# VinAIResearch/DiMSUM

Measured on AMD Instinct MI355X. Metric: denoiser-fwd latents/sec, higher is better.
Workload: dtype f32; 1 GPU; DiM-L/2 denoiser forward, 256px (4x32x32 latents, 256 tokens), 256 latents per GPU, random-init weights (reference init, zero tensors re-drawn N(0, 0.02^2)); global_batch=256, parallelism=dp1 (replicas, independent latents), launch=eager, matmul_policy=f16s (see notes.matmul_policy)

## Files before the change

### dimsum_amd/csrc/xattn_common.hpp

```cpp
#pragma once
#include "common.hpp"

namespace dimsum {

typedef float f4 __attribute__((ext_vector_type(4)));
typedef __bf16 bf16x8 __attribute__((ext_vector_type(8)));
struct alignas(16) u4v { unsigned w[4]; };

__device__ __forceinline__ bf16x8 as_bf16x8(const u4v &v) { return __builtin_bit_cast(bf16x8, v); }

__device__ __forceinline__ float quad_max(float x) {
    auto r = __builtin_amdgcn_permlane16_swap(__float_as_uint(x), __float_as_uint(x), false, false);
    x = fmaxf(__uint_as_float(r[0]), __uint_as_float(r[1]));
    r = __builtin_amdgcn_permlane32_swap(__float_as_uint(x), __float_as_uint(x), false, false);
    return fmaxf(__uint_as_float(r[0]), __uint_as_float(r[1]));
}
__device__ __forceinline__ float quad_sum(float x) {
    auto r = __builtin_amdgcn_permlane16_swap(__float_as_uint(x), __float_as_uint(x), false, false);
    x = __uint_as_float(r[0]) + __uint_as_float(r[1]);
    r = __builtin_amdgcn_permlane32_swap(__float_as_uint(x), __float_as_uint(x), false, false);
    return __uint_as_float(r[0]) + __uint_as_float(r[1]);
}

__device__ __forceinline__ f4 mfma_split(const u4v &ah, const u4v &al, const u4v &bh, const u4v &bl, f4 acc) {
    acc = __builtin_amdgcn_mfma_f32_16x16x32_bf16(as_bf16x8(al), as_bf16x8(bh), acc, 0, 0, 0);
    acc = __builtin_amdgcn_mfma_f32_16x16x32_bf16(as_bf16x8(ah), as_bf16x8(bl), acc, 0, 0, 0);
    acc = __builtin_amdgcn_mfma_f32_16x16x32_bf16(as_bf16x8(ah), as_bf16x8(bh), acc, 0, 0, 0);
    return acc;
}

__device__ __forceinline__ int cslot(int kappa) { return 8 * ((kappa & 15) >> 2) + (kappa & 3) + 4 * (kappa >> 4); }

__device__ __forceinline__ void split_c2(const f4 &t0, const f4 &t1, u4v &hi, u4v &lo) {
    split2(t0[0], t0[1], hi.w[0], lo.w[0]);
    split2(t0[2], t0[3], hi.w[1], lo.w[1]);
    split2(t1[0], t1[1], hi.w[2], lo.w[2]);
    split2(t1[2], t1[3], hi.w[3], lo.w[3]);
}

typedef _Float16 f16x8 __attribute__((ext_vector_type(8)));
__device__ __forceinline__ f16x8 as_f16x8(const u4v &v) { return __builtin_bit_cast(f16x8, v); }
__device__ __forceinline__ unsigned pack_h2(float a, float b) {
    const __half2 h = __floats2half2_rn(a, b);
    return __builtin_bit_cast(unsigned, h);
}
template <bool F16> struct Frag { u4v h, l; };
template <> struct Frag<true> { u4v h; };
template <bool F16> __device__ __forceinline__ void frag_put2(Frag<F16> &f, int i, float x0, float x1) {
    if constexpr (F16) f.h.w[i] = pack_h2(x0, x1);
    else split2(x0, x1, f.h.w[i], f.l.w[i]);
}
template <bool F16> __device__ __forceinline__ Frag<F16> frag_ld(const unsigned short *hi, const unsigned short *lo, int idx) {
    Frag<F16> f;
    f.h = *reinterpret_cast<const u4v *>(&hi[idx]);
    if constexpr (!F16) f.l = *reinterpret_cast<const u4v *>(&lo[idx]);
    return f;
}
template <bool F16> __device__ __forceinline__ f4 frag_mfma(const Frag<F16> &a, const Frag<F16> &b, f4 acc) {
    if constexpr (F16) return __builtin_amdgcn_mfma_f32_16x16x32_f16(as_f16x8(a.h), as_f16x8(b.h), acc, 0, 0, 0);
    else return mfma_split(a.h, a.l, b.h, b.l, acc);
}
template <bool F16> __device__ __forceinline__ Frag<F16> frag_c2(const f4 &t0, const f4 &t1) {
    Frag<F16> f;
    frag_put2<F16>(f, 0, t0[0], t0[1]); frag_put2<F16>(f, 1, t0[2], t0[3]);
    frag_put2<F16>(f, 2, t1[0], t1[1]); frag_put2<F16>(f, 3, t1[2], t1[3]);
    return f;
}
template <bool F16> __device__ __forceinline__ void img_st4(unsigned short *hi, unsigned short *lo, int idx, const float4 &v) {
    if constexpr (F16) *reinterpret_cast<uint2 *>(&hi[idx]) = make_uint2(pack_h2(v.x, v.y), pack_h2(v.z, v.w));
    else {
        unsigned h0, l0, h1, l1;
        split2(v.x, v.y, h0, l0); split2(v.z, v.w, h1, l1);
        *reinterpret_cast<uint2 *>(&hi[idx]) = make_uint2(h0, h1); *reinterpret_cast<uint2 *>(&lo[idx]) = make_uint2(l0, l1);
    }
}
template <bool F16> __device__ __forceinline__ void img_st2(unsigned short *hi, unsigned short *lo, int idx, float x0, float x1) {
    if constexpr (F16) *reinterpret_cast<unsigned *>(&hi[idx]) = pack_h2(x0, x1);
    else {
        unsigned h0, l0;
        split2(x0, x1, h0, l0);
        *reinterpret_cast<unsigned *>(&hi[idx]) = h0; *reinterpret_cast<unsigned *>(&lo[idx]) = l0;
    }
}
template <bool F16> __device__ __forceinline__ void img_zero(unsigned short *hi, unsigned short *lo, int idx) {
    hi[idx] = 0;
    if constexpr (!F16) lo[idx] = 0;
}
__device__ __forceinline__ float row_pow2_scale(float amax) {
    const unsigned e = min((__float_as_uint(amax) >> 23) & 0xffu, 248u);
    return __uint_as_float((249u - e) << 23);
}
constexpr int kPShift = 8;

__device__ __forceinline__ int xcd_group_blocks(int idx, int nblocks, int per_group) {
    if (((nblocks / per_group) & 7) != 0 || nblocks % per_group != 0) return idx;
    const int x = idx & 7, j = idx >> 3;
    return ((j / per_group) * 8 + x) * per_group + (j % per_group);
}

}
```

### dimsum_amd/csrc/xattn_fusion_f16.hip

```cpp
#include <type_traits>

#include "xattn_common.hpp"

namespace dimsum {

constexpr int kKT16 = 64;
constexpr int kQW16 = 16;

template <int HD, int QT, bool kIn16>
__global__ __launch_bounds__(256, (QT == 2 && HD <= 64) ? 3 : 2) void xattn_fusion_fwd_f16_kernel(const dimsum_xattn_params_t p) {
    constexpr int EP = (HD + 31) / 32 * 32;
    constexpr int EC = EP / 32;
    constexpr int ET = (HD + 15) / 16;
    constexpr int KS = EP + 8;
    constexpr int VS = kKT16 + 8;
    static_assert(HD % 8 == 0 && (KS / 8) % 2 == 1 && (VS / 8) % 2 == 1, "layout");
    auto flip = [](int row) { return (((row & 15) + 4) & 8); };
    __shared__ __attribute__((aligned(16))) unsigned short Kh[kKT16 * KS];
    __shared__ __attribute__((aligned(16))) unsigned short Vh[ET * 16 * VS];
    __shared__ float red[8];

    const int tid = threadIdx.x, lane = tid & 63, wave = tid >> 6;
    const int L = p.seqlen, H = p.heads;
    const int qblocks = (L + 64 * QT - 1) / (64 * QT);
    int idx = xcd_group_blocks(blockIdx.x, (int)gridDim.x, qblocks);
    const int qb = idx % qblocks; idx /= qblocks;
    const int ndir = p.n_dirs == 1 ? 1 : 2;
    const int dir = idx % ndir; idx /= ndir;
    const int h = idx % H;
    const int b = idx / H;
    const int C = H * HD;
    const bool kv_from_1 = dir == 1 || ndir == 1;
    using In = typename std::conditional<kIn16, __half, float>::type;
    const In *qsrc = reinterpret_cast<const In *>(dir == 0 ? p.qkv1_ptr : p.qkv2_ptr) + (int64_t)b * p.qkv_batch_stride + h * HD;
    const In *kvsrc = reinterpret_cast<const In *>(kv_from_1 ? p.qkv1_ptr : p.qkv2_ptr) + (int64_t)b * p.qkv_batch_stride + h * HD;
    const In *ksrc = kvsrc + C, *vsrc = kvsrc + 2 * C;
    const int64_t ts = p.qkv_token_stride;
    const float *qbv = reinterpret_cast<const float *>(dir == 0 ? p.bias1_ptr : p.bias2_ptr);
    const float *kvb = reinterpret_cast<const float *>(kv_from_1 ? p.bias1_ptr : p.bias2_ptr);
    const float *qbias = qbv ? qbv + h * HD : nullptr;
    const float *kbias = kvb ? kvb + C + h * HD : nullptr, *vbias = kvb ? kvb + 2 * C + h * HD : nullptr;

    float kv_scale, kv_inv, o_scale = 1.f, o_inv = 1.f;
    const float *bnd = reinterpret_cast<const float *>(p.kv_bound_ptr);
    const float *i1 = reinterpret_cast<const float *>(p.x1_inv_ptr) + (int64_t)b * L;
    const float *i2 = ndir == 2 ? reinterpret_cast<const float *>(p.x2_inv_ptr) + (int64_t)b * L : i1;
    {
        float m1 = 0.f, m2 = 0.f;
        for (int t = tid; t < L; t += 256) { m1 = fmaxf(m1, i1[t]); m2 = fmaxf(m2, i2[t]); }
        m1 = wave_allmax(m1); m2 = wave_allmax(m2);
        if (lane == 0) { red[wave] = m1; red[4 + wave] = m2; }
        __syncthreads();
        m1 = fmaxf(fmaxf(red[0], red[1]), fmaxf(red[2], red[3]));
        m2 = fmaxf(fmaxf(red[4], red[5]), fmaxf(red[6], red[7]));
        const float b1 = 2.0f * (32768.0f * m1 * bnd[0] + bnd[1]), b2 = ndir == 2 ? 2.0f * (32768.0f * m2 * bnd[2] + bnd[3]) : b1;
        f16s_scales(kv_from_1 ? b1 : b2, kv_scale, kv_inv);
        if (p.out_split3 == 2) f16s_scales(fmaxf(b1, b2), o_scale, o_inv);
    }

    const int qi = lane & 15, kg = lane >> 4;
    int q_tok[QT];
    u4v qh[QT][EC];
    float cq[QT];
#pragma unroll
    for (int t = 0; t < QT; ++t) {
        q_tok[t] = qb * (64 * QT) + (wave * QT + t) * kQW16 + qi;
        const int q_ld = min(q_tok[t], L - 1);
        if constexpr (kIn16) {
            float qs, qinv;
            const float xinv = (dir == 0 ? i1 : i2)[q_ld];
            f16s_scales(2.0f * (32768.0f * xinv * bnd[dir == 0 ? 0 : 2] + bnd[dir == 0 ? 1 : 3]), qs, qinv);
            cq[t] = fmaxf(p.scale * kLog2e * qinv * kv_inv, 1.17549435e-38f);
#pragma unroll
            for (int c = 0; c < EC; ++c) {
                const int e0 = 32 * c + 8 * kg;
                qh[t][c] = u4v{{0u, 0u, 0u, 0u}};
                if (e0 < HD) qh[t][c] = *reinterpret_cast<const u4v *>(qsrc + (int64_t)q_ld * ts + e0);
            }
            continue;
        }
        float v[EC][8], qm = 0.f;
#pragma unroll
        for (int c = 0; c < EC; ++c)
#pragma unroll
            for (int half = 0; half < 2; ++half) {
                const int e0 = 32 * c + 8 * kg + 4 * half;
                float4 tq = make_float4(0.f, 0.f, 0.f, 0.f);
                if (e0 < HD) {
                    tq = *reinterpret_cast<const float4 *>(reinterpret_cast<const float *>(qsrc) + (int64_t)q_ld * ts + e0);
                    if (qbias) { const float4 bq = *reinterpret_cast<const float4 *>(qbias + e0); tq.x += bq.x; tq.y += bq.y; tq.z += bq.z; tq.w += bq.w; }
                }
                v[c][4 * half + 0] = tq.x; v[c][4 * half + 1] = tq.y; v[c][4 * half + 2] = tq.z; v[c][4 * half + 3] = tq.w;
                qm = fmaxf(fmaxf(qm, fmaxf(fabsf(tq.x), fabsf(tq.y))), fmaxf(fabsf(tq.z), fabsf(tq.w)));
            }
        float qs, qinv;
        f16s_scales(quad_max(qm), qs, qinv);
        cq[t] = fmaxf(p.scale * kLog2e * qinv * kv_inv, 1.17549435e-38f);
#pragma unroll
        for (int c = 0; c < EC; ++c)
#pragma unroll
            for (int i = 0; i < 4; ++i) qh[t][c].w[i] = pack_h2(v[c][2 * i] * qs, v[c][2 * i + 1] * qs);
    }
    if constexpr (EP > HD) {
        for (int i = tid; i < kKT16 * (EP - HD); i += 256) { const int key = i / (EP - HD), e = (HD + i % (EP - HD)) ^ flip(key); Kh[key * KS + e] = 0; }
    }
    if constexpr (ET * 16 > HD) {
        for (int i = tid; i < (ET * 16 - HD) * kKT16; i += 256) { const int e = HD + i / kKT16, k = (i % kKT16) ^ flip(e); Vh[e * VS + k] = 0; }
    }

    f4 o[QT][ET];
    float m_run[QT], l_run[QT];
#pragma unroll
    for (int t = 0; t < QT; ++t) {
        m_run[t] = -1e30f; l_run[t] = 0.f;
#pragma unroll
        for (int e = 0; e < ET; ++e) o[t][e] = f4{0.f, 0.f, 0.f, 0.f};
    }

    constexpr int kItems = (kKT16 / 2) * (HD / 4), kIters = (kItems + 255) / 256;
    constexpr int kItems16 = (kKT16 / 2) * (HD / 8), kIters16 = (kItems16 + 255) / 256;
    for (int k0 = 0; k0 < L; k0 += kKT16) {
        __syncthreads();
        if constexpr (kIn16) {
#pragma unroll
            for (int it = 0; it < kIters16; ++it) {
                const int i = tid + it * 256;
                if (kItems16 % 256 != 0 && i >= kItems16) continue;
                const int kp = i / (HD / 8), e8 = i - kp * (HD / 8), key = 2 * kp;
                const int tok0 = min(k0 + key, L - 1), tok1 = min(k0 + key + 1, L - 1);
                const u4v ka = *reinterpret_cast<const u4v *>(ksrc + (int64_t)tok0 * ts + e8 * 8), kb = *reinterpret_cast<const u4v *>(ksrc + (int64_t)tok1 * ts + e8 * 8);
                const u4v va = *reinterpret_cast<const u4v *>(vsrc + (int64_t)tok0 * ts + e8 * 8), vb = *reinterpret_cast<const u4v *>(vsrc + (int64_t)tok1 * ts + e8 * 8);
                const int ke = (e8 * 8) ^ flip(key);
                *reinterpret_cast<u4v *>(&Kh[key * KS + ke]) = ka;
                *reinterpret_cast<u4v *>(&Kh[(key + 1) * KS + ke]) = kb;
                const int kap = key & 31, pos = (key & ~31) + 8 * ((kap & 15) >> 2) + (kap & 3) + 4 * (kap >> 4);
#pragma unroll
                for (int j = 0; j < 4; ++j) {
                    *reinterpret_cast<unsigned *>(&Vh[(e8 * 8 + 2 * j) * VS + (pos ^ flip(e8 * 8 + 2 * j))]) = __builtin_amdgcn_perm(vb.w[j], va.w[j], 0x05040100u);
                    *reinterpret_cast<unsigned *>(&Vh[(e8 * 8 + 2 * j + 1) * VS + (pos ^ flip(e8 * 8 + 2 * j + 1))]) = __builtin_amdgcn_perm(vb.w[j], va.w[j], 0x07060302u);
                }
            }
        } else {
#pragma unroll
        for (int it = 0; it < kIters; ++it) {
            const int i = tid + it * 256;
            if (kItems % 256 != 0 && i >= kItems) continue;
            const int kp = i / (HD / 4), e4 = i - kp * (HD / 4), key = 2 * kp;
            const int tok0 = min(k0 + key, L - 1), tok1 = min(k0 + key + 1, L - 1);
            const float *kf = reinterpret_cast<const float *>(ksrc), *vf = reinterpret_cast<const float *>(vsrc);
            float4 ka = *reinterpret_cast<const float4 *>(kf + (int64_t)tok0 * ts + e4 * 4), kb = *reinterpret_cast<const float4 *>(kf + (int64_t)tok1 * ts + e4 * 4);
            float4 va = *reinterpret_cast<const float4 *>(vf + (int64_t)tok0 * ts + e4 * 4), vb = *reinterpret_cast<const float4 *>(vf + (int64_t)tok1 * ts + e4 * 4);
            if (kbias) {
                const float4 bk = *reinterpret_cast<const float4 *>(kbias + e4 * 4), bv = *reinterpret_cast<const float4 *>(vbias + e4 * 4);
                ka.x += bk.x; ka.y += bk.y; ka.z += bk.z; ka.w += bk.w; kb.x += bk.x; kb.y += bk.y; kb.z += bk.z; kb.w += bk.w;
                va.x += bv.x; va.y += bv.y; va.z += bv.z; va.w += bv.w; vb.x += bv.x; vb.y += bv.y; vb.z += bv.z; vb.w += bv.w;
            }
            const int ke = (e4 * 4) ^ flip(key);
            *reinterpret_cast<uint2 *>(&Kh[key * KS + ke]) = make_uint2(pack_h2(ka.x * kv_scale, ka.y * kv_scale), pack_h2(ka.z * kv_scale, ka.w * kv_scale));
            *reinterpret_cast<uint2 *>(&Kh[(key + 1) * KS + ke]) = make_uint2(pack_h2(kb.x * kv_scale, kb.y * kv_scale), pack_h2(kb.z * kv_scale, kb.w * kv_scale));
            const int kap = key & 31, pos = (key & ~31) + 8 * ((kap & 15) >> 2) + (kap & 3) + 4 * (kap >> 4);
            const float a4[4] = {va.x, va.y, va.z, va.w}, b4[4] = {vb.x, vb.y, vb.z, vb.w};
#pragma unroll
            for (int e = 0; e < 4; ++e)
                *reinterpret_cast<unsigned *>(&Vh[(e4 * 4 + e) * VS + (pos ^ flip(e4 * 4))]) = pack_h2(a4[e] * kv_scale, b4[e] * kv_scale);
        }
        }
        __syncthreads();

        f4 s[QT][4];
#pragma unroll
        for (int kt = 0; kt < 4; ++kt) {
            const int krow = (kt * 16 + qi) * KS + ((8 * kg) ^ flip(qi));
#pragma unroll
            for (int t = 0; t < QT; ++t) s[t][kt] = f4{0.f, 0.f, 0.f, 0.f};
#pragma unroll
            for (int c = 0; c < EC; ++c) {
                const u4v kh = *reinterpret_cast<const u4v *>(&Kh[krow + 32 * c]);
#pragma unroll
                for (int t = 0; t < QT; ++t) s[t][kt] = __builtin_amdgcn_mfma_f32_16x16x32_f16(as_f16x8(kh), as_f16x8(qh[t][c]), s[t][kt], 0, 0, 0);
            }
        }
        u4v ph[QT][2];
#pragma unroll
        for (int t = 0; t < QT; ++t) {
            if (k0 + kKT16 > L) {
#pragma unroll
                for (int kt = 0; kt < 4; ++kt)
#pragma unroll
                    for (int r = 0; r < 4; ++r)
                        if (k0 + kt * 16 + kg * 4 + r >= L) s[t][kt][r] = -INFINITY;
            }
            float mx = -INFINITY;
#pragma unroll
            for (int kt = 0; kt < 4; ++kt)
#pragma unroll
                for (int r = 0; r < 4; ++r) mx = fmaxf(mx, s[t][kt][r]);
            mx = quad_max(mx) * cq[t];
            const float m_new = fmaxf(m_run[t], mx);
            const float alpha = fast_exp2(m_run[t] - m_new);
            float rs = 0.f;
#pragma unroll
            for (int kt = 0; kt < 4; ++kt)
#pragma unroll
                for (int r = 0; r < 4; ++r) { s[t][kt][r] = fast_exp2(fmaf(s[t][kt][r], cq[t], -m_new)); rs += s[t][kt][r]; }
            rs = quad_sum(rs);
            l_run[t] = l_run[t] * alpha + rs;
            m_run[t] = m_new;
#pragma unroll
            for (int e = 0; e < ET; ++e) o[t][e] *= alpha;
#pragma unroll
            for (int c = 0; c < 2; ++c) {
                ph[t][c].w[0] = pack_h2(s[t][2 * c][0], s[t][2 * c][1]);
                ph[t][c].w[1] = pack_h2(s[t][2 * c][2], s[t][2 * c][3]);
                ph[t][c].w[2] = pack_h2(s[t][2 * c + 1][0], s[t][2 * c + 1][1]);
                ph[t][c].w[3] = pack_h2(s[t][2 * c + 1][2], s[t][2 * c + 1][3]);
            }
        }
#pragma unroll
        for (int e = 0; e < ET; ++e) {
            const int vrow = (e * 16 + qi) * VS + ((8 * kg) ^ flip(qi));
#pragma unroll
            for (int c = 0; c < 2; ++c) {
                const u4v vh = *reinterpret_cast<const u4v *>(&Vh[vrow + 32 * c]);
#pragma unroll
                for (int t = 0; t < QT; ++t) o[t][e] = __builtin_amdgcn_mfma_f32_16x16x32_f16(as_f16x8(vh), as_f16x8(ph[t][c]), o[t][e], 0, 0, 0);
            }
        }
    }

#pragma unroll
    for (int t = 0; t < QT; ++t) {
        const bool valid = q_tok[t] < L;
        const float inv = kv_inv / l_run[t];
        const int64_t row_off = (int64_t)b * p.out_batch_stride + (int64_t)min(q_tok[t], L - 1) * p.out_token_stride;
        if (p.out_split3 == 2) {
            __half *img = reinterpret_cast<__half *>(p.out_ptr) + row_off + dir * C + h * HD;
            const float sc = inv * o_scale;
            constexpr int kTr = ET >= 4 ? 4 : 0;
            if constexpr (kTr == 4) {
                float x[4][4];
#pragma unroll
                for (int e = 0; e < 4; ++e)
#pragma unroll
                    for (int r = 0; r < 4; ++r) x[e][r] = o[t][e][r] * sc;
#pragma unroll
                for (int r = 0; r < 4; ++r) {
                    { auto q = __builtin_amdgcn_permlane32_swap(__float_as_uint(x[0][r]), __float_as_uint(x[2][r]), false, false); x[0][r] = __uint_as_float(q[0]); x[2][r] = __uint_as_float(q[1]); }
                    { auto q = __builtin_amdgcn_permlane32_swap(__float_as_uint(x[1][r]), __float_as_uint(x[3][r]), false, false); x[1][r] = __uint_as_float(q[0]); x[3][r] = __uint_as_float(q[1]); }
                    { auto q = __builtin_amdgcn_permlane16_swap(__float_as_uint(x[0][r]), __float_as_uint(x[1][r]), false, false); x[0][r] = __uint_as_float(q[0]); x[1][r] = __uint_as_float(q[1]); }
                    { auto q = __builtin_amdgcn_permlane16_swap(__float_as_uint(x[2][r]), __float_as_uint(x[3][r]), false, false); x[2][r] = __uint_as_float(q[0]); x[3][r] = __uint_as_float(q[1]); }
                }
                if (valid) {
                    __half *d0 = img + 16 * kg;
                    *reinterpret_cast<uint4 *>(d0) = make_uint4(pack_h2(x[0][0], x[0][1]), pack_h2(x[0][2], x[0][3]), pack_h2(x[1][0], x[1][1]), pack_h2(x[1][2], x[1][3]));
                    *reinterpret_cast<uint4 *>(d0 + 8) = make_uint4(pack_h2(x[2][0], x[2][1]), pack_h2(x[2][2], x[2][3]), pack_h2(x[3][0], x[3][1]), pack_h2(x[3][2], x[3][3]));
                }
            }
            if (valid) {
#pragma unroll
                for (int e = kTr; e < ET; ++e) {
                    const int e0 = e * 16 + kg * 4;
                    if (e0 < HD) *reinterpret_cast<uint2 *>(img + e0) = make_uint2(pack_h2(o[t][e][0] * sc, o[t][e][1] * sc), pack_h2(o[t][e][2] * sc, o[t][e][3] * sc));
                }
                if (dir == 0 && h == 0 && kg == 0) reinterpret_cast<float *>(p.out_inv_ptr)[(int64_t)b * L + q_tok[t]] = o_inv;
            }
        } else if (valid) {
            float *dst = reinterpret_cast<float *>(p.out_ptr) + row_off + dir * C + h * HD;
#pragma unroll
            for (int e = 0; e < ET; ++e) {
                const int e0 = e * 16 + kg * 4;
                if (e0 < HD) *reinterpret_cast<float4 *>(dst + e0) = make_float4(o[t][e][0] * inv, o[t][e][1] * inv, o[t][e][2] * inv, o[t][e][3] * inv);
            }
        }
        if (valid && p.lse_ptr && kg == 0)
            reinterpret_cast<float *>(p.lse_ptr)[(((int64_t)b * ndir + dir) * H + h) * L + q_tok[t]] = (m_run[t] + __builtin_amdgcn_logf(l_run[t])) * kLn2;
    }
}

int launch_xattn_f16(const dimsum_xattn_params_t &p, hipStream_t s) {
    const bool self_attn = p.n_dirs == 1;
    const bool two = p.seqlen >= 128;
    const int64_t nblk = (int64_t)p.batch * p.heads * (self_attn ? 1 : 2) * ((p.seqlen + (two ? 127 : 63)) / (two ? 128 : 64));
    if (nblk > 0x7fffffff) return DIMSUM_ERR_SHAPE;
    const dim3 grid((unsigned)nblk), block(256);
#define DIMSUM_XF16(HDV)                                                                                \
    if (p.qkv_f16) {                                                                                    \
        if (two) hipLaunchKernelGGL((xattn_fusion_fwd_f16_kernel<HDV, 2, true>), grid, block, 0, s, p); \
        else hipLaunchKernelGGL((xattn_fusion_fwd_f16_kernel<HDV, 1, true>), grid, block, 0, s, p);     \
    } else if (two) hipLaunchKernelGGL((xattn_fusion_fwd_f16_kernel<HDV, 2, false>), grid, block, 0, s, p); \
    else hipLaunchKernelGGL((xattn_fusion_fwd_f16_kernel<HDV, 1, false>), grid, block, 0, s, p)
    switch (p.head_dim) {
        case 24: DIMSUM_XF16(24); break;
        case 32: DIMSUM_XF16(32); break;
        case 48: DIMSUM_XF16(48); break;
        case 64: DIMSUM_XF16(64); break;
        case 72: DIMSUM_XF16(72); break;
        default: return DIMSUM_ERR_SHAPE;
    }
#undef DIMSUM_XF16
    return launch_status();
}

}
```

Measured before the change: 3590 latents/s.

## Store V row-major in LDS and read with ds_read_tr16 transpose loads

V tiles are now written to shared memory in natural key-major layout with a power-of-two XOR swizzle, replacing the scattered per-element transposed stores. The PV MFMA operand is fetched with the hardware transpose-read instruction ds_read_tr16_b64, two loads per fragment. This cuts the staging cost of V (fewer, wider LDS stores, no perm packing) and also raises occupancy to 3 blocks for the f16-input QT=2 variant. The risk is register pressure from the new occupancy bound and bank conflicts if the swizzle does not match the transposed-read pattern.

```diff
diff --git a/dimsum_amd/csrc/xattn_common.hpp b/dimsum_amd/csrc/xattn_common.hpp
--- a/dimsum_amd/csrc/xattn_common.hpp
+++ b/dimsum_amd/csrc/xattn_common.hpp
@@ -1,5 +1,6 @@
 #pragma once
 #include "common.hpp"
+#include "xattn_layout.hpp"
 
 namespace dimsum {
 
@@ -43,6 +44,11 @@
 __device__ __forceinline__ unsigned pack_h2(float a, float b) {
     const __half2 h = __floats2half2_rn(a, b);
     return __builtin_bit_cast(unsigned, h);
+}
+typedef short s16x4 __attribute__((ext_vector_type(4)));
+__device__ __forceinline__ uint2 lds_read_tr16(const unsigned short *p) {
+    typedef __attribute__((address_space(3))) s16x4 lds_s16x4;
+    return __builtin_bit_cast(uint2, __builtin_amdgcn_ds_read_tr16_b64_v4i16((lds_s16x4 *)p));
 }
 template <bool F16> struct Frag { u4v h, l; };
 template <> struct Frag<true> { u4v h; };
diff --git a/dimsum_amd/csrc/xattn_fusion_f16.hip b/dimsum_amd/csrc/xattn_fusion_f16.hip
--- a/dimsum_amd/csrc/xattn_fusion_f16.hip
+++ b/dimsum_amd/csrc/xattn_fusion_f16.hip
@@ -8,16 +8,15 @@
 constexpr int kQW16 = 16;
 
 template <int HD, int QT, bool kIn16>
-__global__ __launch_bounds__(256, (QT == 2 && HD <= 64) ? 3 : 2) void xattn_fusion_fwd_f16_kernel(const dimsum_xattn_params_t p) {
+__global__ __launch_bounds__(256, (QT == 2 && (HD <= 64 || kIn16)) ? 3 : 2) void xattn_fusion_fwd_f16_kernel(const dimsum_xattn_params_t p) {
     constexpr int EP = (HD + 31) / 32 * 32;
     constexpr int EC = EP / 32;
     constexpr int ET = (HD + 15) / 16;
-    constexpr int KS = EP + 8;
-    constexpr int VS = kKT16 + 8;
-    static_assert(HD % 8 == 0 && (KS / 8) % 2 == 1 && (VS / 8) % 2 == 1, "layout");
-    auto flip = [](int row) { return (((row & 15) + 4) & 8); };
+    constexpr int KS = xattn_k_stride(EP);
+    constexpr int VS = xattn_v_stride(ET);
+    static_assert(HD % 8 == 0 && (KS / 8) % 2 == 1 && xattn_v_layout_ok(ET), "layout");
     __shared__ __attribute__((aligned(16))) unsigned short Kh[kKT16 * KS];
-    __shared__ __attribute__((aligned(16))) unsigned short Vh[ET * 16 * VS];
+    __shared__ __attribute__((aligned(16))) unsigned short Vh[kKT16 * VS];
     __shared__ float red[8];
 
     const int tid = threadIdx.x, lane = tid & 63, wave = tid >> 6;
@@ -102,10 +101,10 @@
             for (int i = 0; i < 4; ++i) qh[t][c].w[i] = pack_h2(v[c][2 * i] * qs, v[c][2 * i + 1] * qs);
     }
     if constexpr (EP > HD) {
-        for (int i = tid; i < kKT16 * (EP - HD); i += 256) { const int key = i / (EP - HD), e = (HD + i % (EP - HD)) ^ flip(key); Kh[key * KS + e] = 0; }
+        for (int i = tid; i < kKT16 * (EP - HD); i += 256) { const int key = i / (EP - HD); Kh[xattn_k_idx(EP, key, HD + i % (EP - HD))] = 0; }
     }
     if constexpr (ET * 16 > HD) {
-        for (int i = tid; i < (ET * 16 - HD) * kKT16; i += 256) { const int e = HD + i / kKT16, k = (i % kKT16) ^ flip(e); Vh[e * VS + k] = 0; }
+        for (int i = tid; i < kKT16 * (ET * 16 - HD); i += 256) { const int key = i / (ET * 16 - HD); Vh[xattn_v_idx(ET, key, HD + i % (ET * 16 - HD))] = 0; }
     }
 
     f4 o[QT][ET];
@@ -126,43 +125,35 @@
             for (int it = 0; it < kIters16; ++it) {
                 const int i = tid + it * 256;
                 if (kItems16 % 256 != 0 && i >= kItems16) continue;
-                const int kp = i / (HD / 8), e8 = i - kp * (HD / 8), key = 2 * kp;
+                const int key = xattn_stage16_key(HD, i, 0), e = xattn_stage16_e(HD, i);
                 const int tok0 = min(k0 + key, L - 1), tok1 = min(k0 + key + 1, L - 1);
-                const u4v ka = *reinterpret_cast<const u4v *>(ksrc + (int64_t)tok0 * ts + e8 * 8), kb = *reinterpret_cast<const u4v *>(ksrc + (int64_t)tok1 * ts + e8 * 8);
-                const u4v va = *reinterpret_cast<const u4v *>(vsrc + (int64_t)tok0 * ts + e8 * 8), vb = *reinterpret_cast<const u4v *>(vsrc + (int64_t)tok1 * ts + e8 * 8);
-                const int ke = (e8 * 8) ^ flip(key);
-                *reinterpret_cast<u4v *>(&Kh[key * KS + ke]) = ka;
-                *reinterpret_cast<u4v *>(&Kh[(key + 1) * KS + ke]) = kb;
-                const int kap = key & 31, pos = (key & ~31) + 8 * ((kap & 15) >> 2) + (kap & 3) + 4 * (kap >> 4);
-#pragma unroll
-                for (int j = 0; j < 4; ++j) {
-                    *reinterpret_cast<unsigned *>(&Vh[(e8 * 8 + 2 * j) * VS + (pos ^ flip(e8 * 8 + 2 * j))]) = __builtin_amdgcn_perm(vb.w[j], va.w[j], 0x05040100u);
-                    *reinterpret_cast<unsigned *>(&Vh[(e8 * 8 + 2 * j + 1) * VS + (pos ^ flip(e8 * 8 + 2 * j + 1))]) = __builtin_amdgcn_perm(vb.w[j], va.w[j], 0x07060302u);
-                }
+                const u4v ka = *reinterpret_cast<const u4v *>(ksrc + (int64_t)tok0 * ts + e), kb = *reinterpret_cast<const u4v *>(ksrc + (int64_t)tok1 * ts + e);
+                const u4v va = *reinterpret_cast<const u4v *>(vsrc + (int64_t)tok0 * ts + e), vb = *reinterpret_cast<const u4v *>(vsrc + (int64_t)tok1 * ts + e);
+                *reinterpret_cast<u4v *>(&Kh[xattn_k_idx(EP, key, e)]) = ka;
+                *reinterpret_cast<u4v *>(&Kh[xattn_k_idx(EP, key + 1, e)]) = kb;
+                *reinterpret_cast<u4v *>(&Vh[xattn_v_idx(ET, key, e)]) = va;
+                *reinterpret_cast<u4v *>(&Vh[xattn_v_idx(ET, key + 1, e)]) = vb;
             }
         } else {
 #pragma unroll
         for (int it = 0; it < kIters; ++it) {
             const int i = tid + it * 256;
             if (kItems % 256 != 0 && i >= kItems) continue;
-            const int kp = i / (HD / 4), e4 = i - kp * (HD / 4), key = 2 * kp;
+            const int key = xattn_stage32_key(HD, i, 0), e = xattn_stage32_e(HD, i);
             const int tok0 = min(k0 + key, L - 1), tok1 = min(k0 + key + 1, L - 1);
             const float *kf = reinterpret_cast<const float *>(ksrc), *vf = reinterpret_cast<const float *>(vsrc);
-            float4 ka = *reinterpret_cast<const float4 *>(kf + (int64_t)tok0 * ts + e4 * 4), kb = *reinterpret_cast<const float4 *>(kf + (int64_t)tok1 * ts + e4 * 4);
-            float4 va = *reinterpret_cast<const float4 *>(vf + (int64_t)tok0 * ts + e4 * 4), vb = *reinterpret_cast<const float4 *>(vf + (int64_t)tok1 * ts + e4 * 4);
+            float4 ka = *reinterpret_cast<const float4 *>(kf + (int64_t)tok0 * ts + e), kb = *reinterpret_cast<const float4 *>(kf + (int64_t)tok1 * ts + e);
+            float4 va = *reinterpret_cast<const float4 *>(vf + (int64_t)tok0 * ts + e), vb = *reinterpret_cast<const float4 *>(vf + (int64_t)tok1 * ts + e);
             if (kbias) {
-                const float4 bk = *reinterpret_cast<const float4 *>(kbias + e4 * 4), bv = *reinterpret_cast<const float4 *>(vbias + e4 * 4);
+                const float4 bk = *reinterpret_cast<const float4 *>(kbias + e), bv = *reinterpret_cast<const float4 *>(vbias + e);
                 ka.x += bk.x; ka.y += bk.y; ka.z += bk.z; ka.w += bk.w; kb.x += bk.x; kb.y += bk.y; kb.z += bk.z; kb.w += bk.w;
                 va.x += bv.x; va.y += bv.y; va.z += bv.z; va.w += bv.w; vb.x += bv.x; vb.y += bv.y; vb.z += bv.z; vb.w += bv.w;
             }
-            const int ke = (e4 * 4) ^ flip(key);
-            *reinterpret_cast<uint2 *>(&Kh[key * KS + ke]) = make_uint2(pack_h2(ka.x * kv_scale, ka.y * kv_scale), pack_h2(ka.z * kv_scale, ka.w * kv_scale));
-            *reinterpret_cast<uint2 *>(&Kh[(key + 1) * KS + ke]) = make_uint2(pack_h2(kb.x * kv_scale, kb.y * kv_scale), pack_h2(kb.z * kv_scale, kb.w * kv_scale));
-            const int kap = key & 31, pos = (key & ~31) + 8 * ((kap & 15) >> 2) + (kap & 3) + 4 * (kap >> 4);
-            const float a4[4] = {va.x, va.y, va.z, va.w}, b4[4] = {vb.x, vb.y, vb.z, vb.w};
-#pragma unroll
-            for (int e = 0; e < 4; ++e)
-                *reinterpret_cast<unsigned *>(&Vh[(e4 * 4 + e) * VS + (pos ^ flip(e4 * 4))]) = pack_h2(a4[e] * kv_scale, b4[e] * kv_scale);
+            auto h4 = [&](const float4 &x) { return make_uint2(pack_h2(x.x * kv_scale, x.y * kv_scale), pack_h2(x.z * kv_scale, x.w * kv_scale)); };
+            *reinterpret_cast<uint2 *>(&Kh[xattn_k_idx(EP, key, e)]) = h4(ka);
+            *reinterpret_cast<uint2 *>(&Kh[xattn_k_idx(EP, key + 1, e)]) = h4(kb);
+            *reinterpret_cast<uint2 *>(&Vh[xattn_v_idx(ET, key, e)]) = h4(va);
+            *reinterpret_cast<uint2 *>(&Vh[xattn_v_idx(ET, key + 1, e)]) = h4(vb);
         }
         }
         __syncthreads();
@@ -170,7 +161,7 @@
         f4 s[QT][4];
 #pragma unroll
         for (int kt = 0; kt < 4; ++kt) {
-            const int krow = (kt * 16 + qi) * KS + ((8 * kg) ^ flip(qi));
+            const int krow = xattn_k_read_idx(EP, lane, kt, 0);
 #pragma unroll
             for (int t = 0; t < QT; ++t) s[t][kt] = f4{0.f, 0.f, 0.f, 0.f};
 #pragma unroll
@@ -218,10 +209,10 @@
         }
 #pragma unroll
         for (int e = 0; e < ET; ++e) {
-            const int vrow = (e * 16 + qi) * VS + ((8 * kg) ^ flip(qi));
 #pragma unroll
             for (int c = 0; c < 2; ++c) {
-                const u4v vh = *reinterpret_cast<const u4v *>(&Vh[vrow + 32 * c]);
+                const uint2 v0 = lds_read_tr16(&Vh[xattn_v_read_idx(ET, lane, c, 0, e)]), v1 = lds_read_tr16(&Vh[xattn_v_read_idx(ET, lane, c, 1, e)]);
+                const u4v vh = u4v{{v0.x, v0.y, v1.x, v1.y}};
 #pragma unroll
                 for (int t = 0; t < QT; ++t) o[t][e] = __builtin_amdgcn_mfma_f32_16x16x32_f16(as_f16x8(vh), as_f16x8(ph[t][c]), o[t][e], 0, 0, 0);
             }
diff --git a/dimsum_amd/csrc/xattn_layout.hpp b/dimsum_amd/csrc/xattn_layout.hpp
--- /dev/null
+++ b/dimsum_amd/csrc/xattn_layout.hpp
@@ -0,0 +1,23 @@
+#pragma once
+
+namespace dimsum {
+
+constexpr int xattn_k_stride(int ep) { return ep + 8; }
+constexpr int xattn_k_flip(int row) { return ((row & 15) + 4) & 8; }
+constexpr int xattn_k_idx(int ep, int row, int e) { return row * xattn_k_stride(ep) + (e ^ xattn_k_flip(row)); }
+
+constexpr int xattn_v_stride(int et) { return et * 16; }
+constexpr bool xattn_v_layout_ok(int et) { return et >= 1 && et <= 8 && ((et & 1) == 1 || (et & (et - 1)) == 0); }
+constexpr int xattn_v_swz(int et, int row) { return (et & (et - 1)) == 0 ? ((row * et) >> 3) & (et - 1) : 0; }
+constexpr int xattn_v_idx(int et, int row, int e) { return row * xattn_v_stride(et) + (e ^ (16 * xattn_v_swz(et, row))); }
+
+constexpr int xattn_k_read_idx(int ep, int lane, int kt, int c) { return xattn_k_idx(ep, 16 * kt + (lane & 15), 32 * c + 8 * (lane >> 4)); }
+constexpr int xattn_v_read_idx(int et, int lane, int c, int hf, int et_i) {
+    return xattn_v_idx(et, 32 * c + 16 * hf + 4 * (lane >> 4) + ((lane & 15) >> 2), 16 * et_i + 4 * (lane & 3));
+}
+constexpr int xattn_stage16_key(int hd, int i, int odd) { return 2 * (i / (hd / 8)) + odd; }
+constexpr int xattn_stage16_e(int hd, int i) { return 8 * (i % (hd / 8)); }
+constexpr int xattn_stage32_key(int hd, int i, int odd) { return 2 * (i / (hd / 4)) + odd; }
+constexpr int xattn_stage32_e(int hd, int i) { return 4 * (i % (hd / 4)); }
+
+}
```

Measured after the change: 3597 latents/s (median of 6 runs). Within noise of the previous version (+0.2%).
